# osmocom/osmo-gmr

Hardware: AMD Instinct MI355X
Metric: Mbursts/s demod+Viterbi (and IQ Msamp/s), 1/2/4/8 MI355X (higher is better)
Workload: dtype f32+i32

## Files before the change

### osmo-gmr_amd/csrc/rx_kernels.hip

```cpp
#include <mutex>
#include <type_traits>

#include "gmr1_dev.h"
#include "tch3_body.h"
#include "wave_ops.h"
#include "fast_math.h"

namespace gmr1 {
__constant__ DevBurst c_types[kNumTypes];
}

#include "conv_k5_12.h"
#include "rx_window.h"

namespace gmr1 {

#include "rx_one.h"

__device__ __forceinline__ float2 sync_coef0(const DevBurst &bt, int n, int sps, float fs)
{
	const int nch = bt.n_chunks[0];
	int ch = 0, base = 0, cum = 0;
	for (int c = 0; c < nch - 1; c++) {
		cum += bt.sync[0][c].len;
// ... 352 lines not shown
	typedef Fmt<false> F;
	const DevBurst &bt = c_types[kind ? GMR1_HIP_DC6 : GMR1_HIP_BCCH];
	const int w = in_len - 234 * sps + 1;
	const float2 *__restrict__ in = a.iq + off;
	constexpr int NFULL = (SPS == 4 && NPL == 16) ? 15 : -1;
	constexpr int SIT = SPS == 4 ? 2 : 4;
	float2 wv[NPL];
	float2 sv[3][SIT];
	window_fetch<NPL, NFULL>(in, in_len, lane, wv);
#pragma unroll
	for (int c = 0; c < 3; c++) {
		const int wl = F::clen(bt, kind, c) * sps + w - 1;
		const float2 *__restrict__ src = in + F::cpos(bt, c) * sps;
#pragma unroll
		for (int h = 0; h < SIT; h++) {
			const int sidx = lane + 64 * h;
			sv[c][h] = sidx < wl ? src[sidx] : make_float2(0.f, 0.f);
		}
	}
	if (win) {
#pragma unroll
		for (int k = 0; k < NPL; k++)
			win[lane + 64 * k] = wv[k];
	}
	float avr, avi, inv;
	window_stats<NPL, NFULL>(wv, in_len, lane, avr, avi, inv);
	const float e = window_energy_regs<NPL>(wv, in_len, lane);
	int wb = 0;
#pragma unroll
	for (int c = 0; c < 3; c++) {
		const int wl = F::clen(bt, kind, c) * sps + w - 1;
#pragma unroll
		for (int h = 0; h < SIT; h++) {
			const int sidx = lane + 64 * h;
			if (sidx < wl) {
				const v2f nv = ((v2f){sv[c][h].x, sv[c][h].y} - (v2f){avr, avi}) * (v2f){inv, inv};
				hx[wb + sidx] = make_float2(nv.x, nv.y);
			}
		}
		wb += wl;
	}
	if (lane == 0) {
		hs[0] = avr;
		hs[1] = avi;
		hs[2] = inv;
		hs[3] = e;
	}
}

struct Rx4Cfg {
	static constexpr int NPL = 16, SPS = 4;
	static constexpr bool LAT = false, GEN = false, FAC = false, ACC = false, EN = true, PL = false;
	static constexpr int EBROW = 432, PART = 0;
};
template <int NPL_, int SPS_, bool ACC_, bool EN_, bool PL_ = false>
struct CfgBatch : Rx4Cfg {
	static constexpr int NPL = NPL_, SPS = SPS_;
	static constexpr bool ACC = ACC_, EN = EN_, PL = PL_;
};
template <int NPL_, int SPS_, bool FAC_>
struct CfgDemod : Rx4Cfg {
	static constexpr int NPL = NPL_, SPS = SPS_;
	static constexpr bool GEN = true, FAC = FAC_;
};
struct CfgTch3Front : Rx4Cfg {
	static constexpr int NPL = 8, SPS = 4, EBROW = 216;
	static constexpr bool GEN = true;
};
template <int NPL_, int SPS_, bool ACC_, int PART_ = 0>
struct CfgLoop : Rx4Cfg {
	static constexpr int NPL = NPL_, SPS = SPS_, PART = PART_;
	static constexpr bool LAT = true, ACC = ACC_;
};

template <class P>
struct Rx4Switches : P {
	static constexpr bool SMALL = P::GEN && P::NPL == 8;
	static_assert(!P::FAC || SMALL, "the two-sequence variant builds on the small generic one");
	static_assert(!P::PL || (P::SPS == 4 && !P::GEN && !P::LAT && !P::EN), "the planar layout exists for the fused batch kernel at sps 4");
	static_assert(P::PART == 0 || P::LAT, "only the receive loop's burst is cut in two");
	static constexpr bool PREFETCH_NEXT = P::GEN || P::LAT;
	static constexpr int NSYM = SMALL ? 2 : 4;
	static constexpr int NCHK = SMALL ? 1 : 3;
	static constexpr int NSH = SMALL ? 1 : 2;
	static constexpr bool UB_OVER = !P::LAT && !P::GEN;
	static constexpr bool QL = !P::GEN && !P::LAT && !P::EN && P::SPS == 4 && P::NPL == 16;
	static constexpr bool QX = QL && !P::PL;
	static_assert(!P::PL || QL, "the planar layout exists for the fused batch kernel");
};

template <class Cfg>
__device__ __forceinline__ void rx4_body(const RxArgs &a, const RxIo io, int stage_samples, int cw, int g0, int n_end,
                                         unsigned char *__restrict__ lds_raw, int lane, LatPre<Cfg::NPL, Cfg::SPS> *pre = nullptr)
{
	typedef Rx4Switches<Cfg> C;
	constexpr int NPL = C::NPL, SPS = C::SPS, EBROW = C::EBROW, PART = C::PART;
	constexpr bool LAT = C::LAT, GEN = C::GEN, FAC = C::FAC, ACC = C::ACC, EN = C::EN, PL = C::PL;
	constexpr bool SMALL = C::SMALL, QL = C::QL, QX = C::QX, PREFETCH_NEXT = C::PREFETCH_NEXT, UB_OVER = C::UB_OVER;
	constexpr int NSYM = C::NSYM, NCHK = C::NCHK, NSH = C::NSH;
	const int row = lane >> 4, col = lane & 15;
	const int sps = SPS ? SPS : a.sps;
	const int cwh = FAC ? cw / 2 : cw;
	size_t off[4];
	lds4_layout(stage_samples, cw, off, GEN, UB_OVER, EBROW);
	Lds4 L;
	L.x = reinterpret_cast<float2 *>(lds_raw + off[0]);
	L.corr = reinterpret_cast<float *>(lds_raw + off[1]);
	L.coef = reinterpret_cast<float2 *>(lds_raw + off[2]);
	L.eb = reinterpret_cast<int8_t *>(lds_raw + off[3]);
	L.bm = reinterpret_cast<uint32_t *>(lds_raw + off[0]);
	L.surv = reinterpret_cast<uint64_t *>(lds_raw + off[3]);
	L.ubits = reinterpret_cast<uint32_t *>(lds_raw + off[0] + (UB_OVER ? 0 : 4 * kSteps12 * 4));

	const int g_row = g0 + row;
	const bool row_live = g_row < n_end;

	float avr_r = 0.f, avi_r = 0.f;
	const float2 *xst_lat = L.x;

	float th_q[QX ? 4 : 1][4];
	uint32_t zm_q = 0xff000000u;
	float2 xs_q[2] = {make_float2(0.f, 0.f), make_float2(0.f, 0.f)};
	float inv_r = 1.0f;
	auto op_kind = [&](int g) -> int {
		if constexpr (LAT && PART != 0) return 0; else return io.kind[g] ? 1 : 0;
	};
	auto op_fsh = [&](int g) -> float {
		if constexpr (LAT && PART != 0) return pre->b_fsh; else return io.freq_shift ? io.freq_shift[g] : 0.0f;
	};
	auto op_off = [&](int g) -> uint64_t {
		if constexpr (LAT && PART != 0) return pre->b_off; else return io.offset[g];
	};
	float2 wv_own[NPL];
	bool co_on = false;
	int co_p = 0;
	if constexpr (PART == 2)
		GMR1_STAMP(14);
	else
		GMR1_STAMP(0);
	if constexpr (PART != 2) {
	if constexpr (SMALL) {
		const DevBurst &bt = c_types[a.fixed_type];
		const int in_len = __builtin_amdgcn_readfirstlane(a.in_len[0]);
		const int w = in_len - bt.len * sps + 1;
		const int tl = bt.sync_tl[0];
		const int len0 = bt.sync[0][0].len;
		const int wl = len0 * sps + w - 1;
		const int gq = row_live ? g_row : g0;
		const float2 *__restrict__ in = a.iq + io.offset[gq];
		const float fsh = io.freq_shift ? io.freq_shift[gq] : 0.0f;
		const float fs = (fsh - bt.rotation) / (float)sps;
		float2 *xs = reinterpret_cast<float2 *>(lds_raw) + row * 64;
		L.corr = reinterpret_cast<float *>(lds_raw + 2048);
		float2 *coef = reinterpret_cast<float2 *>(lds_raw + 4096) + row * 16;
		float2 sv[4];
		{
			const float2 *__restrict__ src = in + bt.sync[0][0].pos * sps;
#pragma unroll
			for (int h = 0; h < 4; h++) {
				const int sidx = col + 16 * h;
				sv[h] = sidx < wl ? src[sidx] : make_float2(0.f, 0.f);
			}
		}
		const int nit = in_len >> 4, rem = in_len & 15;
		const bool want_en = io.energy != nullptr;
		v2f s2 = {0.f, 0.f}, q2 = {0.f, 0.f};
#pragma unroll 8
		for (int t = 0; t < nit; t++) {
			const float2 x = in[col + 16 * t];
			s2 += (v2f){x.x, x.y};
			q2 = __builtin_elementwise_fma((v2f){x.x, x.y}, (v2f){x.x, x.y}, q2);
		}
		if (col < rem) {
			const float2 x = in[col + 16 * nit];
			s2 += (v2f){x.x, x.y};
			q2 = __builtin_elementwise_fma((v2f){x.x, x.y}, (v2f){x.x, x.y}, q2);
		}
		float en = 0.f;
		if (want_en) {
			const int bd = in_len >> 5;
			for (int idx = col; idx < in_len; idx += 16)
				if (idx >= bd && idx < in_len - bd) {
					const float2 x = in[idx];
					en = fmaf(x.x, x.x, fmaf(x.y, x.y, en));
				}
// ... 32 lines not shown
				xs[sidx] = make_float2(nv.x, nv.y);
			}
		}
		WSYNC();
		float *corr = L.corr + row * cw;
		for (int j = col; j < w; j += 16) {
			const float2 *xp = xs + j;
			v2f acc0 = {0.f, 0.f}, acc1 = {0.f, 0.f};
			for (int n = 0; n < len0; n++) {
				const float2 x = xp[n * sps];
				const float2 c0 = coef[n];
				acc0 = __builtin_elementwise_fma((v2f){-c0.y, c0.y}, (v2f){x.y, x.x}, acc0);
				acc0 = __builtin_elementwise_fma((v2f){c0.x, c0.x}, (v2f){x.x, x.y}, acc0);
				if constexpr (FAC) {
					const float2 c1 = coef[tl + n];
					acc1 = __builtin_elementwise_fma((v2f){-c1.y, c1.y}, (v2f){x.y, x.x}, acc1);
					acc1 = __builtin_elementwise_fma((v2f){c1.x, c1.x}, (v2f){x.x, x.y}, acc1);
				}
			}
			float cj = 0.f;
			cj += sqrtf(fmaf(acc0.x, acc0.x, acc0.y * acc0.y));
			corr[j] = cj;
			if constexpr (FAC) {
				cj += sqrtf(fmaf(acc1.x, acc1.x, acc1.y * acc1.y));
				corr[cwh + j] = cj;
			}
		}
	} else {
	float2 (&wv)[NPL] = wv_own;
	const int lane_outer = lane;
	int xsp_bc = 0xffff;
	if constexpr (QX) {
		auto place = [&](int kind) -> int {
			const int w = a.in_len[kind] - 234 * 4 + 1;
			const int c0 = kind ? 7 : 11;
			const int n = col;
			const int ch = n < c0 ? 0 : (n < c0 + 3 ? 1 : 2);
			const int nn = n - (ch == 0 ? 0 : (ch == 1 ? c0 : c0 + 3));
			const int wb = ch == 0 ? 0 : (ch == 1 ? c0 * 4 + w - 1 : c0 * 4 + w - 1 + 3 * 4 + w - 1);
			return n < c0 + 6 ? wb + nn * 4 : -1;
		};
		xsp_bc = (place(0) & 0xff) | ((place(1) & 0xff) << 8);
	}
#pragma clang loop unroll_count(QX ? 4 : 1)
	for (int q = 0; q < 4; q++) {
		const int g = g0 + q;
		if (g >= n_end)
			break;
		int lane_l = lane_outer;
		if constexpr (QX)
			asm volatile("" : "+v"(lane_l));
		const int lane = lane_l;
		const int row = lane >> 4, col = lane & 15;
		const int kind = GEN ? 0 : __builtin_amdgcn_readfirstlane(op_kind(g));
		const int type = GEN ? a.fixed_type : (kind ? GMR1_HIP_DC6 : GMR1_HIP_BCCH);
		const int in_len = __builtin_amdgcn_readfirstlane(a.in_len[kind]);
		const DevBurst &bt = c_types[type];
		typedef Fmt<GEN> F;
		const int w = in_len - F::len(bt) * sps + 1;
		const float fsh = op_fsh(g);
		const float fs = (fsh - F::rotation(bt)) / (float)sps;

		const float2 *__restrict__ in = a.iq + op_off(g);
		const int sl = lane;
		const int tl = F::tl(bt, kind);
		const int nch = F::nch(bt);
		constexpr int NFULL = (!GEN && SPS == 4 && NPL == 16) ? 15 : -1;
		constexpr int SIT = SMALL ? 1 : (SPS == 4 ? 2 : 4);
		float2 sv_own[NCHK][SIT];
		float2 (&sv)[NCHK][SIT] = sv_own;
		auto fetch_window = [&](const float2 *__restrict__ from) {
			window_fetch<NPL, NFULL>(from, in_len, lane, wv);
#pragma unroll
			for (int c = 0; c < NCHK; c++) {
				const int wl = c < nch ? F::clen(bt, kind, c) * sps + w - 1 : 0;
				const float2 *__restrict__ src = from + (c < nch ? F::cpos(bt, c) * sps : 0);
#pragma unroll
				for (int h = 0; h < SIT; h++) {
					const int sidx = lane + 64 * h;
					sv[c][h] = sidx < wl ? src[sidx] : make_float2(0.f, 0.f);
				}
			}
		};
		bool prepared = false;
		const float2 *__restrict__ xst = L.x;
		if constexpr (LAT) {
			prepared = *pre->h_off == op_off(g) && *pre->h_kind == kind;
			if (prepared)
				xst = xst_lat = pre->h_x;
			if constexpr (PART == 1)
				co_on = prepared && pre->co != nullptr && kind == 0;
		}
		if (LAT) {
			if (!prepared)
				fetch_window(in);
		} else {
			if constexpr (PL) {
				window_fetch_q_planar(a.iq, a.plane_stride, io.offset[g], in_len, lane, wv);
			} else {
			if constexpr (QL)
				window_fetch_q(in, in_len, lane, wv);
			else if (q == 0 || !PREFETCH_NEXT)
				window_fetch<NPL, NFULL>(in, in_len, lane, wv);
#pragma unroll
			for (int c = 0; c < NCHK; c++) {
				const int wl = c < nch ? F::clen(bt, kind, c) * sps + w - 1 : 0;
				const float2 *__restrict__ src = in + (c < nch ? F::cpos(bt, c) * sps : 0);
#pragma unroll
				for (int h = 0; h < SIT; h++) {
					const int sidx = lane + 64 * h;
					sv[c][h] = sidx < wl ? src[sidx] : make_float2(0.f, 0.f);
				}
			}
			}
		}
		float2 cfl = make_float2(0.f, 0.f);
		const float2 *__restrict__ ctab = (!GEN && io.freq_shift == nullptr) ? c_coef0[sps][type] : nullptr;
		if (io.freq_shift == nullptr) {
			if (GEN && lane < 32)
				cfl = g_coef0[sps][type][lane];
		} else if (lane < tl) {
			if constexpr (GEN) {
				cfl = sync_coef0(bt, lane, sps, fs);
			} else {
				cfl = lat_coef(kind, lane, fs, sps);
			}
		}
		WSYNC();
		if constexpr (FAC) {
			if (lane < 2 * tl)
				L.coef[lane] = sync_coef_seq1(bt, lane >= tl ? 1 : 0, lane >= tl ? lane - tl : lane, sps, fs);
		} else if (GEN && lane < tl)
			L.coef[lane] = cfl;
		float avr, avi, inv;
		if (prepared) {
			avr = pre->h_stat[0];
			avi = pre->h_stat[1];
			inv = pre->h_stat[2];
			if constexpr (PART == 1)
				pre->out_energy = pre->h_stat[3];
			if (io.energy && lane == 0)
				io.energy[g] = pre->h_stat[3];
		} else {
		if constexpr (QL)
			window_stats_q(wv, in_len, lane, avr, avi, inv);
		else
			window_stats<NPL, NFULL>(wv, in_len, sl, avr, avi, inv, -1, 1);
		if constexpr (LAT && PART == 1) {
			if (pre->win_w) {
#pragma unroll
				for (int k = 0; k < NPL; k++)
					pre->win_w[lane + 64 * k] = wv[k];
			}
		}
		if constexpr (LAT && PART == 1) {
			const float e = window_energy_regs<NPL>(wv, in_len, lane);
			pre->out_energy = e;
			if (io.energy && lane == 0)
				io.energy[g] = e;
		} else if ((LAT || !PREFETCH_NEXT) && EN && io.energy) {
			const float e = window_energy_regs<NPL>(wv, in_len, lane);
			if (lane == 0)
				io.energy[g] = e;
		}
		}
		GMR1_STAMP(1);
		if (row == q) { avr_r = avr; avi_r = avi; inv_r = inv; }
		if (PREFETCH_NEXT && !LAT && q + 1 < 4 && g + 1 < n_end) {
			const int kind1 = GEN ? 0 : __builtin_amdgcn_readfirstlane(io.kind[g + 1] ? 1 : 0);
			window_fetch<NPL, NFULL>(a.iq + io.offset[g + 1], __builtin_amdgcn_readfirstlane(a.in_len[kind1]), lane, wv);
		}
		if (!LAT && PREFETCH_NEXT && EN && io.energy) {
			const float e = window_energy<NPL>(in, in_len, lane);
			if (lane == 0)
				io.energy[g] = e;
		}
		if constexpr (PL) {
			const int wl0 = F::clen(bt, kind, 0) * 4 + w - 1, wl1 = 3 * 4 + w - 1;
			const v2f av = {avr, avi}, iv = {inv, inv};
			auto stage_quad = [&](int b, int start, int wl, int wb) {
				const int rel = 256 * b + 4 * lane - start;
				if (rel >= 0 && rel < wl) {
					v2f n0 = ((v2f){wv[4 * b].x, wv[4 * b].y} - av) * iv, n1 = ((v2f){wv[4 * b + 1].x, wv[4 * b + 1].y} - av) * iv;
					v2f n2 = ((v2f){wv[4 * b + 2].x, wv[4 * b + 2].y} - av) * iv, n3 = ((v2f){wv[4 * b + 3].x, wv[4 * b + 3].y} - av) * iv;
					float4 *dst = reinterpret_cast<float4 *>(L.x + wb + rel);
					dst[0] = make_float4(n0.x, n0.y, n1.x, n1.y);
					dst[1] = make_float4(n2.x, n2.y, n3.x, n3.y);
				}
			};
			stage_quad(0, 28 * 4, wl0, 0);
			stage_quad(1, 119 * 4, wl1, wl0);
			stage_quad(2, 119 * 4, wl1, wl0);
			stage_quad(3, 197 * 4, wl1, wl0 + wl1);
		} else
		if (!prepared) {
			int wb = 0;
#pragma unroll
			for (int c = 0; c < NCHK; c++) {
				const int wl = c < nch ? F::clen(bt, kind, c) * sps + w - 1 : 0;
#pragma unroll
				for (int h = 0; h < SIT; h++) {
					const int sidx = sl + 64 * h;
					if (sidx < wl) {
						const v2f nv = ((v2f){sv[c][h].x, sv[c][h].y} - (v2f){avr, avi}) * (v2f){inv, inv};
						L.x[wb + sidx] = make_float2(nv.x, nv.y);
					}
				}
				wb += wl;
			}
		}
		WSYNC();
		float *corr = L.corr + q * cw;
		if constexpr (!GEN) {
			if (LAT && PART == 1 && co_on) {
				const int j0 = ((w - 1) >> 6) << 6;
				corr_fixed<SPS, 11, 3, 3>(xst, sps, w, lane, ctab, cfl, corr, 0, j0);
				if (lds_wait_eq(&pre->co->c_id, pre->co_id)) {
					if (lane < w - j0)
						corr[j0 + lane] = pre->co->tail[lane];
				} else
					corr_fixed<SPS, 11, 3, 3>(xst, sps, w, lane, ctab, cfl, corr, j0, w);
			} else if constexpr (QX) {
				uint32_t cbest = 0;
				int cbj = 0;
				if (kind == 0)
					corr_fixed<SPS, 11, 3, 3>(xst, sps, w, lane, ctab, cfl, corr, 0, -1, &cbest, &cbj);
				else
					corr_fixed<SPS, 7, 3, 3>(xst, sps, w, lane, ctab, cfl, corr, 0, -1, &cbest, &cbj);
				uint32_t mx = cbest, o;
				o = dpp<0xB1>(mx); mx = o > mx ? o : mx;
				o = dpp<0x4E>(mx); mx = o > mx ? o : mx;
				o = dpp<0x141>(mx); mx = o > mx ? o : mx;
				o = dpp<0x140>(mx); mx = o > mx ? o : mx;
				const uint32_t m01 = max((uint32_t)__builtin_amdgcn_readlane((int)mx, 0), (uint32_t)__builtin_amdgcn_readlane((int)mx, 16));
				const uint32_t m23 = max((uint32_t)__builtin_amdgcn_readlane((int)mx, 32), (uint32_t)__builtin_amdgcn_readlane((int)mx, 48));
				const uint32_t M = max(m01, m23);
				const unsigned long long holders = __ballot(cbest == M);
				const int d = __builtin_amdgcn_readlane(cbj, holders ? __builtin_ctzll(holders) : 0);
				if (row == q) {
					zm_q = (zm_q & 0x00ffffffu) | ((uint32_t)d << 24);
					const int pl = (xsp_bc >> (kind ? 8 : 0)) & 0xff;
					if (pl != 0xff)
						xs_q[0] = xst[pl + d];
					if (kind == 0 && col == 0)
						xs_q[1] = xst[11 * 4 + w - 1 + 3 * 4 + w - 1 + 2 * 4 + d];
				}
				{
					const int srcl = lane + (d >> 2);
					const int addr = (srcl & 63) << 2;
					const bool up = srcl >= 64;
					float2 rot[4];
					auto pull = [&](const float2 &v) {
						return make_float2(__builtin_bit_cast(float, __builtin_amdgcn_ds_bpermute(addr, __builtin_bit_cast(int, v.x))),
						                   __builtin_bit_cast(float, __builtin_amdgcn_ds_bpermute(addr, __builtin_bit_cast(int, v.y))));
					};
					switch (d & 3) {
					case 0: rot[0] = pull(wv[0]); rot[1] = pull(wv[4]); rot[2] = pull(wv[8]); rot[3] = pull(wv[12]); break;
					case 1: rot[0] = pull(wv[1]); rot[1] = pull(wv[5]); rot[2] = pull(wv[9]); rot[3] = pull(wv[13]); break;
					case 2: rot[0] = pull(wv[2]); rot[1] = pull(wv[6]); rot[2] = pull(wv[10]); rot[3] = pull(wv[14]); break;
					default: rot[0] = pull(wv[3]); rot[1] = pull(wv[7]); rot[2] = pull(wv[11]); rot[3] = pull(wv[15]); break;
					}
#pragma unroll
					for (int r = 0; r < 4; r++) {
// ... 2 lines not shown
						const bool ok = r < 3 || (i < 234 && 4 * i + d < in_len);
						x.x -= avr;
						x.y -= avi;
						th_q[q][r] = atan2_turns(x.y, x.x);
						if (!ok || (x.x == 0.0f && x.y == 0.0f))
							zm_q |= 1u << (4 * q + r);
					}
				}
			} else if (kind == 0)
				corr_fixed<SPS, 11, 3, 3>(xst, sps, w, lane, ctab, cfl, corr);
			else
				corr_fixed<SPS, 7, 3, 3>(xst, sps, w, lane, ctab, cfl, corr);
		} else if constexpr (FAC) {
			const int len = bt.sync[0][0].len;
			for (int j = lane; j < w; j += 64) {
				const float2 *xp = L.x + j;
				v2f acc0 = {0.f, 0.f}, acc1 = {0.f, 0.f};
				for (int n = 0; n < len; n++) {
					const float2 x = xp[n * sps];
					const float2 c0 = L.coef[n], c1 = L.coef[tl + n];
					acc0 = __builtin_elementwise_fma((v2f){-c0.y, c0.y}, (v2f){x.y, x.x}, acc0);
					acc0 = __builtin_elementwise_fma((v2f){c0.x, c0.x}, (v2f){x.x, x.y}, acc0);
					acc1 = __builtin_elementwise_fma((v2f){-c1.y, c1.y}, (v2f){x.y, x.x}, acc1);
					acc1 = __builtin_elementwise_fma((v2f){c1.x, c1.x}, (v2f){x.x, x.y}, acc1);
				}
				float cj = 0.f;
				cj += sqrtf(fmaf(acc0.x, acc0.x, acc0.y * acc0.y));
				corr[j] = cj;
				cj += sqrtf(fmaf(acc1.x, acc1.x, acc1.y * acc1.y));
				corr[cwh + j] = cj;
			}
		} else
		for (int j = lane; j < w; j += 64) {
			float cj = 0.f;
			int base = 0, wb = 0;
			for (int ch = 0; ch < nch; ch++) {
				const int len = F::clen(bt, kind, ch);
				const float2 *xp = L.x + wb + j;
				const float2 *cp = L.coef + base;
				v2f acc = {0.f, 0.f};
				for (int n = 0; n < len; n++) {
					const float2 x = xp[n * sps];
					const float2 cf = cp[n];
					acc = __builtin_elementwise_fma((v2f){-cf.y, cf.y}, (v2f){x.y, x.x}, acc);
					acc = __builtin_elementwise_fma((v2f){cf.x, cf.x}, (v2f){x.x, x.y}, acc);
				}
				const float ar = acc.x, ai = acc.y;
				base += len;
				wb += len * sps + w - 1;
				cj += sqrtf(fmaf(ar, ar, ai * ai));
			}
			corr[j] = cj;
		}
	}
	}
	WSYNC();
	GMR1_STAMP(2);
	if (a.dbg_stop == 2) return;
	}

	const int kind_r = (!GEN && row_live) ? op_kind(g_row) : 0;
	const int type_r = GEN ? a.fixed_type : (kind_r ? GMR1_HIP_DC6 : GMR1_HIP_BCCH);
	typedef Fmt<GEN> F;
	const int in_len_r = kind_r ? a.in_len[1] : a.in_len[0];
	const float fsh_r = row_live ? op_fsh(g_row) : 0.0f;
	const DevBurst &bt_r = c_types[type_r];
	const float fs_r = (fsh_r - F::rotation(bt_r)) / (float)sps;
	const int w_r = in_len_r - F::len(bt_r) * sps + 1;
	const float2 *__restrict__ in_r = a.iq + (row_live ? op_off(g_row) : 0);

	const float *cr = L.corr + (LAT ? 0 : row) * cw;
	const int w_p = LAT ? __builtin_amdgcn_readlane(w_r, 0) : w_r;
	const int tl_p = LAT ? F::tl(c_types[__builtin_amdgcn_readlane(type_r, 0)], __builtin_amdgcn_readlane(kind_r, 0)) : F::tl(bt_r, kind_r);
	const int win = LAT ? 3 : (w_p < 3 ? w_p : 3);
	const bool w3 = !LAT && __ballot(win != 3) == 0;
	float toa_r = 0.f, p_pwr = 0.f;
	int sid_r = -1;
	if constexpr (PART == 2) {
		toa_r = pre->cut->toa;
		sid_r = pre->cut->sid;
		avr_r = pre->cut->avr;
		avi_r = pre->cut->avi;
	}
	for (int sq = 0; sq < (PART == 2 ? 0 : (FAC ? 2 : 1)); sq++) {
		if (FAC)
			cr = L.corr + row * cw + sq * cwh;
		GMR1_STAMP(10);
		int mi;
		if constexpr (LAT) {
			constexpr int NH = SPS == 4 ? 2 : 3;
			uint32_t eb2[NH];
			bool ok2[NH];
			uint32_t mx = 0;
#pragma unroll
			for (int h = 0; h < NH; h++) {
				const int m = lane + 64 * h;
				ok2[h] = m + win <= w_p;
				float e = 0.f;
				for (int k = 0; k < win; k++) {
					const float c = cr[ok2[h] ? m + k : 0];
					e += c * c;
				}
				eb2[h] = ok2[h] ? __builtin_bit_cast(uint32_t, e) : 0u;
				mx = eb2[h] > mx ? eb2[h] : mx;
			}
			uint32_t o;
			o = dpp<0xB1>(mx); mx = o > mx ? o : mx;
			o = dpp<0x4E>(mx); mx = o > mx ? o : mx;
			o = dpp<0x141>(mx); mx = o > mx ? o : mx;
			o = dpp<0x140>(mx); mx = o > mx ? o : mx;
			const uint32_t m01 = max((uint32_t)__builtin_amdgcn_readlane((int)mx, 0), (uint32_t)__builtin_amdgcn_readlane((int)mx, 16));
			const uint32_t m23 = max((uint32_t)__builtin_amdgcn_readlane((int)mx, 32), (uint32_t)__builtin_amdgcn_readlane((int)mx, 48));
			const uint32_t M = max(m01, m23);
			mi = 0;
#pragma unroll
			for (int h = NH - 1; h >= 0; h--) {
				const unsigned long long bh = __ballot(ok2[h] && eb2[h] == M);
				if (bh)
					mi = 64 * h + __builtin_ctzll(bh);
			}
		} else {
		if (w3) {
// ... 387 lines not shown
					f += atan2_fast(im, re) / (cpos - ppos);
				}
			}
			ffe_r = f / (float)(nch_r - 1);
		}
		float tr = 0.f, ti = 0.f;
#pragma unroll
		for (int h = 0; h < NSH; h++) {
			float2 tt = t0[h];
			if (ffe_r != 0.0f) {
				float s, c;
				sincos_fast(-ffe_r * (float)spos[h], s, c);
				tt = cmul(tt, make_float2(c, s));
			}
			tr += tt.x;
			ti += tt.y;
		}
		psi_r = atan2_fast(row_sum(ti), row_sum(tr));
	}
	if constexpr (PART != 2) {
	GMR1_STAMP(4);
	if (a.dbg_stop == 5) return;

	if (col == 0 && row_live && (PART != 1 || io.rv)) {
		const int rv = found_r ? 0 : -1;
		io.rv[g_row] = rv;
		if (io.sync_id) io.sync_id[g_row] = found_r ? sid_r : -1;
		if (io.toa) io.toa[g_row] = found_r ? toa_r : 0.f;
		if (io.freq_err) io.freq_err[g_row] = found_r ? ffe_r : 0.f;
	}
	}
	if constexpr (PART == 1) {
		auto first_f = [](float v) { return __builtin_bit_cast(float, __builtin_amdgcn_readfirstlane(__builtin_bit_cast(int, v))); };
		pre->out = {__builtin_amdgcn_readfirstlane(found_r ? 1 : 0), __builtin_amdgcn_readfirstlane(d_r), __builtin_amdgcn_readfirstlane(sid_r),
		            first_f(found_r ? toa_r : 0.f), first_f(found_r ? ffe_r : 0.f), first_f(psi_r), first_f(avr_r), first_f(avi_r)};
		if (lane == 0)
			*pre->cut = {found_r ? 1 : 0, d_r, sid_r, toa_r, ffe_r, psi_r, avr_r, avi_r};
		return;
	}

	const unsigned char *lut = lds_raw + (GEN ? 4 * EBROW : 0);
	if constexpr (LAT) {
		lut = pre->lut;
		WSYNC();
	} else {
		unsigned char *const lutw = lds_raw + (GEN ? 4 * EBROW : 0);
		const uint4 *__restrict__ lut_src = reinterpret_cast<const uint4 *>(FAC ? g_sb_lut1.v : g_sb_lut.v);
		const uint4 lut_a = lut_src[lane], lut_b = lut_src[lane + 64];
		WSYNC();
		reinterpret_cast<uint4 *>(lutw)[lane] = lut_a;
		reinterpret_cast<uint4 *>(lutw)[lane + 64] = lut_b;
		WSYNC();
	}
	int row_ok = 0, row_chain = 0;
	Sym4 nxt1, nxt2;
	if constexpr (!QX) { nxt1 = first; nxt2 = second; }
#pragma unroll
	for (int q = 3; q >= 0; q--) {
		const int g = g0 + q;
		Sym4 cur;
		if constexpr (LAT) {
			if (q != 0)
				continue;
			cur = first;
		} else if constexpr (QX) {
			cur.ok = 0;
#pragma unroll
			for (int r = 0; r < NSYM; r++) cur.x[r] = make_float2(0.f, 0.f);
		} else {
			cur = nxt1;
			nxt1 = nxt2;
			fetch(q - 2, nxt2);
		}
		if (g >= n_end)
			continue;
		const int src = 16 * q;
		const bool hit = QX && __builtin_amdgcn_readlane((int)hit_r, src) != 0;
		if constexpr (QX) {
			if (!hit && __builtin_amdgcn_readlane((int)found_r, src) != 0) {
				if (q == first_q)
					cur = first;
				else
					fetch(q, cur);
			}
		}
		const bool found = __builtin_amdgcn_readlane((int)found_r, src) != 0;
		const int kind = __builtin_amdgcn_readlane(kind_r, src);
		const int type = GEN ? a.fixed_type : (kind ? GMR1_HIP_DC6 : GMR1_HIP_BCCH);
		const DevBurst &bt = c_types[type];
		const int d = __builtin_amdgcn_readlane(d_r, src);
		const float fs = lane_val(fs_r, src);
		const float rps = -lane_val(ffe_r, src);
		const float psi = lane_val(psi_r, src);
		const float avr = lane_val(avr_r, src), avi = lane_val(avi_r, src);
		const int blen = F::len(bt), nbits = F::nbits(bt);
		float *gss = io.ssyms ? io.ssyms + (size_t)g * a.ssyms_stride : nullptr;
		int8_t *eb = L.eb + q * (GEN ? EBROW : 432);
		row_chain |= kind << q;
		if (!found) {
			if (io.ebits)
				for (int i = lane; i < a.ebits_stride; i += 64)
					io.ebits[(size_t)g * a.ebits_stride + i] = 0;
			if constexpr (GEN)
				for (int i = lane; i < EBROW / 4; i += 64)
					reinterpret_cast<uint32_t *>(eb)[i] = 0;
			if (gss)
// ... 96 lines not shown
	GMR1_STAMP(7);
	if (col == 0 && row_live) {
		if ((row_ok >> row) & 1) {
			store_l2(io.l2 + (size_t)g_row * 24, L.ubits + row * 8);
			io.crc[g_row] = syn ? 1 : 0;
			io.conv[g_row] = (int32_t)fae;
		} else {
			uint32_t *l2w = reinterpret_cast<uint32_t *>(io.l2 + (size_t)g_row * 24);
#pragma unroll
			for (int i = 0; i < 6; i++)
				l2w[i] = 0;
			io.crc[g_row] = -1;
			io.conv[g_row] = 0;
		}
	}
}

#ifndef GMR1_EXP_RX4_WAVES
#define GMR1_EXP_RX4_WAVES 6
#endif
template <int NPL, int SPS, bool EN = false>
constexpr int kRx4Waves = NPL > 16 ? 3 : ((SPS == 4 && !EN) ? GMR1_EXP_RX4_WAVES : 5);

template <int NPL, int SPS, bool ACC = false, bool EN = false, bool PL = false>
__global__ __launch_bounds__(64) __attribute__((amdgpu_waves_per_eu(kRx4Waves<NPL, SPS, EN>, kRx4Waves<NPL, SPS, EN>)))
void k_rx4(RxArgs a, int stage_samples, int cw, int bpw)
{
	extern __shared__ __align__(16) unsigned char lds_raw[];
	int g0 = blockIdx.x * bpw;
	int n_end = min(a.n, g0 + bpw);
	if (EN && a.seg_count) {
		int sg = g0 / a.seg_stride;
		int lo = 0;
		if (a.seg_first) {
			if (a.seg_groups > 0) {
				sg = (int)blockIdx.x / a.seg_groups;
				lo = (a.seg_first[sg] + 3) & ~3;
				g0 = sg * a.seg_stride + lo + ((int)blockIdx.x % a.seg_groups) * bpw;
			} else {
				lo = (a.seg_first[sg] + 3) & ~3;
			}
		}
		const int base = sg * a.seg_stride;
		n_end = min(min(a.n, g0 + bpw), base + min(a.seg_count[sg], a.seg_stride));
		if (g0 >= n_end || g0 < base + lo)
			return;
	}
	const RxIo io = {
#ifdef GMR1_HIP_PROFILE
	                 nullptr,
#endif
	                 a.offset, a.kind, a.freq_shift, a.l2, a.crc, a.conv, a.rv, a.sync_id, a.toa, a.freq_err, a.energy,
	                 a.ebits, a.ssyms};
	rx4_body<CfgBatch<NPL, SPS, ACC, EN, PL>>(a, io, stage_samples, cw, g0, n_end, lds_raw, (int)threadIdx.x);
}

template <int NPL, int SPS, bool FAC = false>
__global__ __launch_bounds__(64) void k_rx4g(RxArgs a, int stage_samples, int cw)
{
	extern __shared__ __align__(16) unsigned char lds_raw[];
	const int g0 = blockIdx.x * 4;
	const RxIo io = {
#ifdef GMR1_HIP_PROFILE
	                 nullptr,
#endif
	                 a.offset, nullptr, a.freq_shift, nullptr, nullptr, nullptr, a.rv, a.sync_id, a.toa, a.freq_err, a.energy,
	                 a.ebits, a.ssyms};
	rx4_body<CfgDemod<NPL, SPS, FAC>>(a, io, stage_samples, cw, g0, min(a.n, g0 + 4), lds_raw, (int)threadIdx.x);
}

template <bool ACC>
constexpr int kRx4gTch3Waves = 7;
template <bool ACC>
__global__ __launch_bounds__(64) __attribute__((amdgpu_waves_per_eu(kRx4gTch3Waves<ACC>, kRx4gTch3Waves<ACC>))) void k_rx4g_tch3(RxArgs a, Tch3Args t, int stage_samples, int cw)
{
	extern __shared__ __align__(16) unsigned char lds_raw[];
	const int g0 = blockIdx.x * 4;
	const int lane = (int)threadIdx.x;
	const int n_end = min(a.n, g0 + 4);
	const RxIo io = {
#ifdef GMR1_HIP_PROFILE
	                 nullptr,
#endif
	                 a.offset, nullptr, a.freq_shift, nullptr, nullptr, nullptr, a.rv, a.sync_id, a.toa, a.freq_err, a.energy,
	                 a.ebits, a.ssyms};
	constexpr int kRow = 216;
	static_assert(CfgTch3Front::EBROW == kRow, "the body's soft-bit rows are the decoder's");
	rx4_body<CfgTch3Front>(a, io, stage_samples, cw, g0, n_end, lds_raw, lane);
	t3::Tch3Lds *S = reinterpret_cast<t3::Tch3Lds *>(lds_raw + 4 * kRow);
	WSYNC();
	t3::tch3_fill_locof(S, lane);
	if (lane < 4)
		*reinterpret_cast<uint32_t *>(lds_raw + lane * kRow + 212) = 0;
	t3::Tch3Lane lc;
	t3::tch3_lane(lc, S, lane);
	WSYNC();
	for (int q = 0; q < 4 && g0 + q < n_end; q++) {
		t3::tch3_burst<ACC>(t, g0 + q, lane, reinterpret_cast<const int8_t *>(lds_raw + q * kRow), S, lc);
		WSYNC();
	}
}

#include "rx_small_kernels.h"

template <int NPL, int SPS>
static hipError_t launch_rx_t(const RxArgs &a, bool decode, int max_in_len, int max_len, hipStream_t stream)
{
// ... 145 lines not shown
```

### osmo-gmr_amd/csrc/rx_window.h

```cpp
#pragma once
#include "conv_k5_12.h"

namespace gmr1 {

static constexpr int kEbRow = 448;
static constexpr int kEbitsLds = 704;

struct Lds {
	float2 *x;
	float *corr;
	float2 *coef;
	float2 *y;
	int8_t *eb;
	uint32_t *bm;
	uint64_t *surv;
	uint32_t *ubits;
};

__host__ __device__ inline size_t align16(size_t v) { return (v + 15) & ~(size_t)15; }

__host__ __device__ inline size_t lds_corr_bytes(int max_len, bool decode)
{
	if (decode)
		return align16((size_t)max_len * 4);
	return align16((size_t)(max_len > kMaxWindow ? max_len : kMaxWindow) * 4);
}

__host__ __device__ inline size_t lds_layout(int max_in_len, int max_len, bool decode, size_t *off)
{
	size_t o = 0;
	size_t xbytes = align16((size_t)max_in_len * 8);
	const size_t dec_bytes = 4 * kSteps12 * 4 + kSteps12 * 8 + 4 * 8 * 4;
	if (decode && xbytes < dec_bytes)
		xbytes = align16(dec_bytes);
	off[0] = o; o += xbytes;
	const size_t corr_bytes = lds_corr_bytes(max_len, decode);
	const size_t coef_bytes = decode ? 32 * 8 : (size_t)kMaxCoef * 8;
	off[1] = o; o += corr_bytes + coef_bytes;
	off[2] = o; o += decode ? 4 * kEbRow : kEbitsLds;
	return align16(o);
}

__device__ __forceinline__ Lds lds_carve(unsigned char *raw, int max_in_len, int max_len, bool decode)
{
	size_t off[3];
	lds_layout(max_in_len, max_len, decode, off);
	Lds L;
	L.x = reinterpret_cast<float2 *>(raw + off[0]);
	L.corr = reinterpret_cast<float *>(raw + off[1]);
	L.coef = reinterpret_cast<float2 *>(raw + off[1] + lds_corr_bytes(max_len, decode));
	L.y = reinterpret_cast<float2 *>(raw + off[1]);
	L.eb = reinterpret_cast<int8_t *>(raw + off[2]);
	L.bm = reinterpret_cast<uint32_t *>(raw + off[0]);
	L.surv = reinterpret_cast<uint64_t *>(raw + off[0] + 4 * kSteps12 * 4);
// ... 61 lines not shown
			v[k] = in[l0 + RS * k];
		else if (k == nfull && tail)
			v[k] = in[l0 + RS * k];
		else
			v[k] = make_float2(0.f, 0.f);
	}
}

template <int NPL, int NFULL = -1>
__device__ __forceinline__ void window_stats(const float2 (&v)[NPL], int in_len, int lane,
                                             float &avr_o, float &avi_o, float &inv_o, int perm_src = -1, int odd_src = 1)
{
	auto home = [&](float x) {
		return perm_src < 0 ? x : __builtin_bit_cast(float, __builtin_amdgcn_ds_bpermute(perm_src << 2, __builtin_bit_cast(int, x)));
	};
	v2f s2 = {0.f, 0.f};
	const int nfull = NFULL >= 0 ? NFULL : (in_len >> 6);
	const bool tail = (lane + 64 * nfull) < in_len;
#pragma unroll
	for (int k = 0; k < NPL; k++)
		s2 += (v2f){v[k].x, v[k].y};
	const float sr = wave_sum(home(s2.x));
	const float si = wave_sum(home(s2.y));
	const float inv_n = __builtin_amdgcn_rcpf((float)in_len);
	const float quot = ((lane & 1) ? si : sr) / (float)in_len;
	const float avr = lane_val(quot, 0), avi = lane_val(quot, odd_src);
	const v2f av = {avr, avi};
	v2f acc2 = {0.f, 0.f};
#pragma unroll
	for (int k = 0; k < NPL; k++) {
		if (k < nfull || (k == nfull && tail)) {
			const v2f d = (v2f){v[k].x, v[k].y} - av;
			acc2 = __builtin_elementwise_fma(d, d, acc2);
		}
	}
	float stddev = __builtin_amdgcn_sqrtf(wave_sum(home(acc2.x + acc2.y)) * inv_n);
	if (stddev == 0.0f)
		stddev = 1.0f;
	avr_o = avr;
	avi_o = avi;
	inv_o = __builtin_amdgcn_rcpf(stddev);
}

template <int NPL, int NFULL = -1>
__device__ __forceinline__ void load_stats(const float2 *__restrict__ in, int in_len, int lane,
                                           float &avr_o, float &avi_o, float &inv_o)
{
	float2 v[NPL];
	window_fetch<NPL, NFULL>(in, in_len, lane, v);
	window_stats<NPL, NFULL>(v, in_len, lane, avr_o, avi_o, inv_o);
}

typedef float v4f_a8 __attribute__((ext_vector_type(4), aligned(8)));
__device__ __forceinline__ void window_fetch_q(const float2 *__restrict__ in, int in_len, int lane, float2 (&v)[16])
{
	const v4f_a8 *__restrict__ p = reinterpret_cast<const v4f_a8 *>(in + 4 * lane);
#pragma unroll
	for (int b = 0; b < 4; b++) {
		const int s0 = 256 * b + 4 * lane;
#pragma unroll
		for (int h = 0; h < 2; h++) {
			float2 lo = make_float2(0.f, 0.f), hi = make_float2(0.f, 0.f);
			if (b < 3 || s0 + 2 * h + 1 < in_len) {
				const v4f_a8 u = p[128 * b + h];
				lo = make_float2(u.x, u.y);
				hi = make_float2(u.z, u.w);
			} else if (s0 + 2 * h < in_len) {
				lo = in[s0 + 2 * h];
			}
			v[4 * b + 2 * h] = lo;
			v[4 * b + 2 * h + 1] = hi;
		}
	}
}

__device__ __forceinline__ void window_fetch_q_planar(const float2 *__restrict__ pl, long long plane_stride, uint64_t o, int in_len,
                                                      int lane, float2 (&v)[16])
{
#pragma unroll
	for (int c = 0; c < 4; c++) {
		const uint64_t oc = o + (uint64_t)c;
		const float2 *__restrict__ src = pl + (long long)(oc & 3) * plane_stride + (long long)(oc >> 2) + lane;
#pragma unroll
		for (int b = 0; b < 4; b++) {
			const int sidx = 256 * b + 4 * lane + c;
			v[4 * b + c] = (b < 3 || sidx < in_len) ? src[64 * b] : make_float2(0.f, 0.f);
		}
	}
}

__device__ __forceinline__ void window_stats_q(const float2 (&v)[16], int in_len, int lane, float &avr_o, float &avi_o, float &inv_o)
{
	v2f s2 = {0.f, 0.f}, q2 = {0.f, 0.f};
#pragma unroll
	for (int k = 0; k < 16; k++) {
		const v2f x = {v[k].x, v[k].y};
		s2 += x;
		q2 = __builtin_elementwise_fma(x, x, q2);
	}
	const float sr = wave_sum(s2.x);
	const float si = wave_sum(s2.y);
	const float sq = wave_sum(q2.x + q2.y);
	const float inv_n = __builtin_amdgcn_rcpf((float)in_len);
	const float quot = ((lane & 1) ? si : sr) / (float)in_len;
	const float avr = lane_val(quot, 0), avi = lane_val(quot, 1);
	const float var = fmaxf(fmaf(-(float)in_len, fmaf(avr, avr, avi * avi), sq), 0.0f) * inv_n;
	float stddev = __builtin_amdgcn_sqrtf(var);
	if (stddev == 0.0f)
		stddev = 1.0f;
	avr_o = avr;
	avi_o = avi;
	inv_o = __builtin_amdgcn_rcpf(stddev);
}

template <int NPL>
__device__ __noinline__ float window_energy(const float2 *__restrict__ in, int in_len, int lane)
{
	const int bd = in_len >> 5;
	float e = 0.f;
#pragma unroll
	for (int k = 0; k < NPL; k++) {
		const int idx = lane + 64 * k;
		if (idx >= bd && idx < in_len - bd) {
			const float2 v = in[idx];
			e = fmaf(v.x, v.x, fmaf(v.y, v.y, e));
		}
// ... 27 lines not shown
```

Before: 449.3.

## Hoist per-burst metadata loads ahead and unify tail window load

For the fused batch kernel, loads kind, offset and frequency shift for all four bursts up front, makes them wave-uniform, and reuses them in both the per-burst loop and the per-row phase. This removes repeated dependent global loads of metadata from the inner loop. The last window block becomes a single vector load, with a shifted load plus register fix-up for a partial tail. An optional experimental touch of the next burst's window lines is added but is off by default (TOUCH=0). The gains rest on shorter load latency chains, and the tail shuffle adds a little work.

```diff
diff --git a/osmo-gmr_amd/csrc/rx_kernels.hip b/osmo-gmr_amd/csrc/rx_kernels.hip
--- a/osmo-gmr_amd/csrc/rx_kernels.hip
+++ b/osmo-gmr_amd/csrc/rx_kernels.hip
@@ -428,11 +428,12 @@
 	static constexpr int NPL = 16, SPS = 4;
 	static constexpr bool LAT = false, GEN = false, FAC = false, ACC = false, EN = true, PL = false;
 	static constexpr int EBROW = 432, PART = 0;
+	static constexpr bool EARLY = false;
 };
-template <int NPL_, int SPS_, bool ACC_, bool EN_, bool PL_ = false>
+template <int NPL_, int SPS_, bool ACC_, bool EN_, bool PL_ = false, bool EARLY_ = false>
 struct CfgBatch : Rx4Cfg {
 	static constexpr int NPL = NPL_, SPS = SPS_;
-	static constexpr bool ACC = ACC_, EN = EN_, PL = PL_;
+	static constexpr bool ACC = ACC_, EN = EN_, PL = PL_, EARLY = EARLY_;
 };
 template <int NPL_, int SPS_, bool FAC_>
 struct CfgDemod : Rx4Cfg {
@@ -449,6 +450,10 @@
 	static constexpr bool LAT = true, ACC = ACC_;
 };
 
+#ifndef GMR1_EXP_RX4_TOUCH
+#define GMR1_EXP_RX4_TOUCH 0
+#endif
+
 template <class P>
 struct Rx4Switches : P {
 	static constexpr bool SMALL = P::GEN && P::NPL == 8;
@@ -463,6 +468,9 @@
 	static constexpr bool QL = !P::GEN && !P::LAT && !P::EN && P::SPS == 4 && P::NPL == 16;
 	static constexpr bool QX = QL && !P::PL;
 	static_assert(!P::PL || QL, "the planar layout exists for the fused batch kernel");
+	static constexpr bool AHEAD = P::EARLY && QX;
+	static constexpr int TOUCH = AHEAD ? GMR1_EXP_RX4_TOUCH : 0;
+	static constexpr bool H_ROW = AHEAD, ONE_LOAD = AHEAD;
 };
 
 template <class Cfg>
@@ -474,6 +482,8 @@
 	constexpr bool LAT = C::LAT, GEN = C::GEN, FAC = C::FAC, ACC = C::ACC, EN = C::EN, PL = C::PL;
 	constexpr bool SMALL = C::SMALL, QL = C::QL, QX = C::QX, PREFETCH_NEXT = C::PREFETCH_NEXT, UB_OVER = C::UB_OVER;
 	constexpr int NSYM = C::NSYM, NCHK = C::NCHK, NSH = C::NSH;
+	constexpr int TOUCH = C::TOUCH;
+	constexpr bool AHEAD = C::AHEAD, H_ROW = C::H_ROW;
 	const int row = lane >> 4, col = lane & 15;
 	const int sps = SPS ? SPS : a.sps;
 	const int cwh = FAC ? cw / 2 : cw;
@@ -507,6 +517,30 @@
 	auto op_off = [&](int g) -> uint64_t {
 		if constexpr (LAT && PART != 0) return pre->b_off; else return io.offset[g];
 	};
+	int kind_s[4] = {0, 0, 0, 0};
+	uint64_t off_s[4] = {0, 0, 0, 0};
+	float fsh_s[4] = {0.f, 0.f, 0.f, 0.f};
+	if constexpr (AHEAD) {
+		if (g0 < n_end) {
+			int kv[4];
+			uint64_t ov[4];
+			float fv[4];
+#pragma unroll
+			for (int q = 0; q < 4; q++) {
+				const int gq = g0 + q < n_end ? g0 + q : g0;
+				kv[q] = op_kind(gq);
+				ov[q] = op_off(gq);
+				fv[q] = op_fsh(gq);
+			}
+#pragma unroll
+			for (int q = 0; q < 4; q++) {
+				kind_s[q] = __builtin_amdgcn_readfirstlane(kv[q]);
+				off_s[q] = (uint64_t)(uint32_t)__builtin_amdgcn_readfirstlane((int)(uint32_t)ov[q]) |
+				           ((uint64_t)(uint32_t)__builtin_amdgcn_readfirstlane((int)(uint32_t)(ov[q] >> 32)) << 32);
+				fsh_s[q] = __builtin_bit_cast(float, __builtin_amdgcn_readfirstlane(__builtin_bit_cast(int, fv[q])));
+			}
+		}
+	}
 	float2 wv_own[NPL];
 	bool co_on = false;
 	int co_p = 0;
@@ -645,16 +679,32 @@
 			asm volatile("" : "+v"(lane_l));
 		const int lane = lane_l;
 		const int row = lane >> 4, col = lane & 15;
-		const int kind = GEN ? 0 : __builtin_amdgcn_readfirstlane(op_kind(g));
+		const bool has_nx = TOUCH != 0 && window_touch_wanted(q, g, n_end);
+		int kind_l;
+		if constexpr (AHEAD)
+			kind_l = kind_s[q];
+		else
+			kind_l = GEN ? 0 : __builtin_amdgcn_readfirstlane(op_kind(g));
+		const int kind = kind_l;
 		const int type = GEN ? a.fixed_type : (kind ? GMR1_HIP_DC6 : GMR1_HIP_BCCH);
 		const int in_len = __builtin_amdgcn_readfirstlane(a.in_len[kind]);
 		const DevBurst &bt = c_types[type];
 		typedef Fmt<GEN> F;
 		const int w = in_len - F::len(bt) * sps + 1;
-		const float fsh = op_fsh(g);
+		float fsh_l;
+		if constexpr (AHEAD)
+			fsh_l = fsh_s[q];
+		else
+			fsh_l = op_fsh(g);
+		const float fsh = fsh_l;
 		const float fs = (fsh - F::rotation(bt)) / (float)sps;
 
-		const float2 *__restrict__ in = a.iq + op_off(g);
+		const float2 *__restrict__ in = a.iq + (AHEAD ? off_s[q] : op_off(g));
+		Touched touched = {0, 0};
+		auto touch_next = [&]() {
+			if (has_nx)
+				touched = window_touch_q(a.iq + off_s[(q + 1) & 3], __builtin_amdgcn_readfirstlane(a.in_len[kind_s[(q + 1) & 3]]), lane);
+		};
 		const int sl = lane;
 		const int tl = F::tl(bt, kind);
 		const int nch = F::nch(bt);
@@ -692,7 +742,7 @@
 				window_fetch_q_planar(a.iq, a.plane_stride, io.offset[g], in_len, lane, wv);
 			} else {
 			if constexpr (QL)
-				window_fetch_q(in, in_len, lane, wv);
+				window_fetch_q<C::ONE_LOAD>(in, in_len, lane, wv);
 			else if (q == 0 || !PREFETCH_NEXT)
 				window_fetch<NPL, NFULL>(in, in_len, lane, wv);
 #pragma unroll
@@ -705,6 +755,10 @@
 					sv[c][h] = sidx < wl ? src[sidx] : make_float2(0.f, 0.f);
 				}
 			}
+			if constexpr (TOUCH == 1)
+				touch_next();
+			if constexpr (C::ONE_LOAD)
+				window_fix_q(in_len, lane, wv);
 			}
 		}
 		float2 cfl = make_float2(0.f, 0.f);
@@ -759,6 +813,8 @@
 		}
 		GMR1_STAMP(1);
 		if (row == q) { avr_r = avr; avi_r = avi; inv_r = inv; }
+		if constexpr (TOUCH == 2)
+			touch_next();
 		if (PREFETCH_NEXT && !LAT && q + 1 < 4 && g + 1 < n_end) {
 			const int kind1 = GEN ? 0 : __builtin_amdgcn_readfirstlane(io.kind[g + 1] ? 1 : 0);
 			window_fetch<NPL, NFULL>(a.iq + io.offset[g + 1], __builtin_amdgcn_readfirstlane(a.in_len[kind1]), lane, wv);
@@ -802,6 +858,8 @@
 				wb += wl;
 			}
 		}
+		if constexpr (TOUCH == 1)
+			window_touch_done(touched);
 		WSYNC();
 		float *corr = L.corr + q * cw;
 		if constexpr (!GEN) {
@@ -910,6 +968,8 @@
 			}
 			corr[j] = cj;
 		}
+		if constexpr (TOUCH == 2)
+			window_touch_done(touched);
 	}
 	}
 	WSYNC();
@@ -917,15 +977,41 @@
 	if (a.dbg_stop == 2) return;
 	}
 
-	const int kind_r = (!GEN && row_live) ? op_kind(g_row) : 0;
+
+	int kind_row = 0;
+	uint64_t off_row = 0;
+	float fsh_row = 0.f;
+	if constexpr (H_ROW) {
+		int row_o = row;
+		asm volatile("" : "+v"(row_o));
+		kind_row = row_o == 0 ? kind_s[0] : (row_o == 1 ? kind_s[1] : (row_o == 2 ? kind_s[2] : kind_s[3]));
+		off_row = row_o == 0 ? off_s[0] : (row_o == 1 ? off_s[1] : (row_o == 2 ? off_s[2] : off_s[3]));
+		fsh_row = row_o == 0 ? fsh_s[0] : (row_o == 1 ? fsh_s[1] : (row_o == 2 ? fsh_s[2] : fsh_s[3]));
+		if (!row_live) {
+			kind_row = 0;
+			off_row = 0;
+			fsh_row = 0.f;
+		}
+	}
+	int kind_r_l;
+	if constexpr (H_ROW)
+		kind_r_l = kind_row;
+	else
+		kind_r_l = (!GEN && row_live) ? op_kind(g_row) : 0;
+	const int kind_r = kind_r_l;
 	const int type_r = GEN ? a.fixed_type : (kind_r ? GMR1_HIP_DC6 : GMR1_HIP_BCCH);
 	typedef Fmt<GEN> F;
 	const int in_len_r = kind_r ? a.in_len[1] : a.in_len[0];
-	const float fsh_r = row_live ? op_fsh(g_row) : 0.0f;
+	float fsh_r_l;
+	if constexpr (H_ROW)
+		fsh_r_l = fsh_row;
+	else
+		fsh_r_l = row_live ? op_fsh(g_row) : 0.0f;
+	const float fsh_r = fsh_r_l;
 	const DevBurst &bt_r = c_types[type_r];
 	const float fs_r = (fsh_r - F::rotation(bt_r)) / (float)sps;
 	const int w_r = in_len_r - F::len(bt_r) * sps + 1;
-	const float2 *__restrict__ in_r = a.iq + (row_live ? op_off(g_row) : 0);
+	const float2 *__restrict__ in_r = a.iq + (H_ROW ? off_row : (row_live ? op_off(g_row) : 0));
 
 	const float *cr = L.corr + (LAT ? 0 : row) * cw;
 	const int w_p = LAT ? __builtin_amdgcn_readlane(w_r, 0) : w_r;
@@ -1419,6 +1505,7 @@
 		reinterpret_cast<uint4 *>(lutw)[lane + 64] = lut_b;
 		WSYNC();
 	}
+
 	int row_ok = 0, row_chain = 0;
 	Sym4 nxt1, nxt2;
 	if constexpr (!QX) { nxt1 = first; nxt2 = second; }
@@ -1621,7 +1708,7 @@
 #endif
 	                 a.offset, a.kind, a.freq_shift, a.l2, a.crc, a.conv, a.rv, a.sync_id, a.toa, a.freq_err, a.energy,
 	                 a.ebits, a.ssyms};
-	rx4_body<CfgBatch<NPL, SPS, ACC, EN, PL>>(a, io, stage_samples, cw, g0, n_end, lds_raw, (int)threadIdx.x);
+	rx4_body<CfgBatch<NPL, SPS, ACC, EN, PL, true>>(a, io, stage_samples, cw, g0, n_end, lds_raw, (int)threadIdx.x);
 }
 
 template <int NPL, int SPS, bool FAC = false>
diff --git a/osmo-gmr_amd/csrc/rx_touch.h b/osmo-gmr_amd/csrc/rx_touch.h
--- /dev/null
+++ b/osmo-gmr_amd/csrc/rx_touch.h
@@ -0,0 +1,29 @@
+#pragma once
+#include <stdint.h>
+
+#if defined(__HIPCC__)
+#define GMR1_TOUCH_HD __host__ __device__
+#else
+#define GMR1_TOUCH_HD
+#endif
+
+namespace gmr1 {
+
+static constexpr int kTouchLine = 128;
+static constexpr int kTouchSlots = 65;
+
+GMR1_TOUCH_HD inline bool window_touch_wanted(int q, int g, int n_end)
+{
+	return q < 3 && g + 1 < n_end;
+}
+
+GMR1_TOUCH_HD inline int window_touch_offset(unsigned misalign, int in_len, int slot)
+{
+	if (slot < 0 || slot >= kTouchSlots || in_len <= 0)
+		return -1;
+	const int last = 8 * in_len - 4;
+	const int o = slot == 0 ? 0 : kTouchLine * slot - (int)(misalign & (unsigned)(kTouchLine - 1));
+	return o <= last ? o : -1;
+}
+
+}
diff --git a/osmo-gmr_amd/csrc/rx_window.h b/osmo-gmr_amd/csrc/rx_window.h
--- a/osmo-gmr_amd/csrc/rx_window.h
+++ b/osmo-gmr_amd/csrc/rx_window.h
@@ -1,5 +1,6 @@
 #pragma once
 #include "conv_k5_12.h"
+#include "rx_touch.h"
 
 namespace gmr1 {
 
@@ -167,6 +168,7 @@
 }
 
 typedef float v4f_a8 __attribute__((ext_vector_type(4), aligned(8)));
+template <bool ONE = false>
 __device__ __forceinline__ void window_fetch_q(const float2 *__restrict__ in, int in_len, int lane, float2 (&v)[16])
 {
 	const v4f_a8 *__restrict__ p = reinterpret_cast<const v4f_a8 *>(in + 4 * lane);
@@ -176,6 +178,14 @@
 #pragma unroll
 		for (int h = 0; h < 2; h++) {
 			float2 lo = make_float2(0.f, 0.f), hi = make_float2(0.f, 0.f);
+			if (ONE && b == 3) {
+				const bool full = s0 + 2 * h + 1 < in_len, part = !full && s0 + 2 * h < in_len;
+				if (full || part) {
+					const v4f_a8 u = *reinterpret_cast<const v4f_a8 *>(in + s0 + 2 * h - (part ? 1 : 0));
+					lo = make_float2(u.x, u.y);
+					hi = make_float2(u.z, u.w);
+				}
+			} else
 			if (b < 3 || s0 + 2 * h + 1 < in_len) {
 				const v4f_a8 u = p[128 * b + h];
 				lo = make_float2(u.x, u.y);
@@ -187,6 +197,36 @@
 			v[4 * b + 2 * h + 1] = hi;
 		}
 	}
+}
+
+__device__ __forceinline__ void window_fix_q(int in_len, int lane, float2 (&v)[16])
+{
+	const int s0 = 256 * 3 + 4 * lane;
+#pragma unroll
+	for (int h = 0; h < 2; h++) {
+		const bool part = s0 + 2 * h + 1 >= in_len && s0 + 2 * h < in_len;
+		v[12 + 2 * h] = part ? v[12 + 2 * h + 1] : v[12 + 2 * h];
+		v[12 + 2 * h + 1] = part ? make_float2(0.f, 0.f) : v[12 + 2 * h + 1];
+	}
+}
+
+struct Touched { uint32_t a, b; };
+__device__ __forceinline__ Touched window_touch_q(const float2 *__restrict__ next, int in_len, int lane)
+{
+	const char *base = reinterpret_cast<const char *>(next);
+	const unsigned mis = (unsigned)(reinterpret_cast<uintptr_t>(next) & (uintptr_t)(kTouchLine - 1));
+	const int o = window_touch_offset(mis, in_len, lane);
+	Touched t = {0, 0};
+	if (o >= 0)
+		t.a = *reinterpret_cast<const uint32_t *>(base + o);
+	const int o64 = window_touch_offset(mis, in_len, 64);
+	if (o64 >= 0 && lane == 0)
+		t.b = *reinterpret_cast<const uint32_t *>(base + o64);
+	return t;
+}
+__device__ __forceinline__ void window_touch_done(const Touched &t)
+{
+	asm volatile("" : : "v"(t.a), "v"(t.b));
 }
 
 __device__ __forceinline__ void window_fetch_q_planar(const float2 *__restrict__ pl, long long plane_stride, uint64_t o, int in_len,
```

New measurement: 468.6 (median of 6 runs). 1.04x the previous value.
